# Joao-M-Silva/padel_analytics

Hardware: AMD Instinct MI355X
Metric: frames/sec (all trackers) on 1280x720 (higher is better)
Workload: dtype f32-equivalent (h2: fp16 pairs h + m/2048, 2 or 3 f16 MFMA products per multiply, fp32 accumulate)

## Files before the change

padel_analytics_amd/csrc/conv_1x1_h2s.hip:

```cpp
#include "h2_common.h"

namespace padel {

namespace {

}

#ifndef PADEL_HS_AWIN
#define PADEL_HS_AWIN D
#endif
template <int WC, int PROBE = 0, int D = 2, int WR = 2>
__global__ void __launch_bounds__(64 * WR * WC, 2) conv_h2s_kernel(const ConvArgs a) {
    constexpr int MF = 4, NF = 3, NSET = D + 1;
    constexpr int kSPlaneB = 64 * WR * 64;
    constexpr int kSStageB = 2 * kSPlaneB;
    constexpr int kSStages = WC == 2 ? 5 : 9;
    constexpr int kSAhead = kSStages - 1;
    constexpr int NA = 8 / (2 * WC) * 2;
    static_assert(WR == 2 || WC == 4, "64-pixel tiles: one span per wave");
    __shared__ __attribute__((aligned(16))) float lds[(kSStages * kSStageB) / 4];
    char* const ldsb = reinterpret_cast<char*>(lds);
    const int tid = threadIdx.x;
    const int lane = tid & 63;
    const int wave = __builtin_amdgcn_readfirstlane(tid >> 6);
    const int wr = WR == 2 ? (wave & 1) : 0, wc = WR == 2 ? (wave >> 1) : wave;
    const int lr = lane & 15, lq = lane >> 4;

    const int nmt = a.n_mtiles, nnt = a.n_ntiles;
    const int bid = blockIdx.x;
    const XcdSlot slot = xcd_slot(nmt, nnt, bid);
    if (xcd_slot_padding(slot)) return;
    const int mt = xcd_slot_mtile(slot), nt = slot.nt;
    const int m0 = mt * (64 * WR);
    const int f0 = nt * WC * NF;
    const int nch = a.cin >> 5;

    const long long pix_b = (long long)a.in_cs * 4;
    const char* const in0 = reinterpret_cast<const char*>(a.in + a.in_choff) + (long long)m0 * pix_b;
    i32x4 rsrcA = make_rsrc(in0);
    {
        const long long left = ((long long)a.M - m0) * pix_b;
        rsrcA[2] = (int)(left > 0x7FFFFFFFll ? 0x7FFFFFFFll : left);
    }
    const int p_q = (lane & 3) ^ (((lane >> 4) & 1) << 1);
    const unsigned p_piece = (unsigned)((p_q >> 1) * 64 + (p_q & 1) * 16);
    unsigned voA[2];
#pragma unroll
    for (int k = 0; k < 2; ++k) voA[k] = (unsigned)(((wave + 4 * k) * 16 + (lane >> 2)) * (unsigned)pix_b) + p_piece;
    unsigned voL[2];
#pragma unroll
    for (int k = 0; k < 2; ++k) voL[k] = (unsigned)((wave * 16 + 8 * k + (lane >> 3)) * (unsigned)pix_b) + (unsigned)(lane & 7) * 16u;
    i32x4 sink[2] = {};
    unsigned voQ[2];
#pragma unroll
    for (int k = 0; k < 2; ++k) voQ[k] = (unsigned)(wave * 2048 + k * 1024 + lane * 16);
    const unsigned lp0 = __builtin_amdgcn_readfirstlane((unsigned)(uintptr_t)lds);
    const unsigned lpw = __builtin_amdgcn_readfirstlane(lp0 + (unsigned)wave * 1024u);
#define PADEL_HS_REQA(SB_, K_)                                                                                    \
    if constexpr (PROBE != 3) {                                                                                   \
        const unsigned so_ = (unsigned)(K_) * 128u;                                                               \
        const unsigned lb_ = lpw + (unsigned)(SB_);                                                               \
        i32x4 rs_ = rsrcA;                                                                                        \
        if ((int)(K_) >= nch) rs_[2] = 0;                                                                         \
        if constexpr (PROBE == 4) { lds_dma<0>(voL[0], rs_, so_, lb_); lds_dma<kSPlaneB>(voL[1], rs_, so_, lb_); } \
        else if constexpr (PROBE == 6) {                                                                          \
            asm volatile("buffer_load_dwordx4 %0, %1, %2, %3 offen" : "=v"(sink[0]) : "v"(voA[0]), "s"(rs_), "s"(so_) : "memory"); \
            asm volatile("buffer_load_dwordx4 %0, %1, %2, %3 offen" : "=v"(sink[1]) : "v"(voA[0]), "s"(rs_), "s"(so_ + 32u) : "memory"); \
        }                                                                                                         \
        else if constexpr (PROBE == 5) { lds_dma<0>(voQ[0], rs_, so_ * 128u, lb_); lds_dma<kSPlaneB>(voQ[1], rs_, so_ * 128u, lb_); } \
        else {                                                                                                    \
        lds_dma<0>(voA[0], rs_, so_, lb_); if constexpr (WC == 2) lds_dma<4096>(voA[1], rs_, so_, lb_);           \
        lds_dma<kSPlaneB>(voA[0], rs_, so_ + 32u, lb_); if constexpr (WC == 2) lds_dma<kSPlaneB + 4096>(voA[1], rs_, so_ + 32u, lb_); \
        }                                                                                                         \
    }

    const unsigned fragb = (unsigned)nch * 2048u;
    const unsigned voffW = (unsigned)lane * 16u;
    i32x4 rsrcW[NF];
#pragma unroll
    for (int j = 0; j < NF; ++j) {
        const int frag = min(f0 + NF * wc + j, a.n16 - 1);
        rsrcW[j] = make_rsrc(reinterpret_cast<const char*>(a.wr) + (long long)frag * fragb);
    }
    i32x4 w[NSET][NF];
#define PADEL_HS_LOADW(SET_, K_)                                                                                  \
    if constexpr (PROBE != 2 && PROBE < 4 || PROBE == 7) {                                                        \
        const unsigned so_ = (unsigned)(K_) * 2048u;                                                              \
        if (PROBE == 7 && wr == 1) rsrcW[0][2] = rsrcW[1][2] = rsrcW[2][2] = 0;      \
        _Pragma("unroll") for (int j = 0; j < NF; ++j)                                                            \
            asm volatile("buffer_load_dwordx4 %0, %1, %2, %3 offen" : "=v"(w[SET_][j]) : "v"(voffW), "s"(rsrcW[j]), "s"(so_) : "memory"); \
    }
#define PADEL_HS_WAITW(SET_, N_)                                                                                  \
    asm volatile("s_waitcnt vmcnt(%3)" : "+v"(w[SET_][0]), "+v"(w[SET_][1]), "+v"(w[SET_][2]) : "n"(PROBE == 2 || (PROBE >= 4 && PROBE != 7) ? ((N_) == 0 ? 0 : (PADEL_HS_AWIN) * NA) : PROBE == 3 ? (N_) * NF / (NF + NA) : (N_)) : "memory")

    const unsigned abase = swz_off(64 * wr + lr, lq);
    f32x4 acc[MF][NF], part[MF][NF], cross[MF][NF];
#pragma unroll
    for (int f = 0; f < MF; ++f)
#pragma unroll
        for (int j = 0; j < NF; ++j) { acc[f][j] = (f32x4){0.f, 0.f, 0.f, 0.f}; part[f][j] = acc[f][j]; cross[f][j] = acc[f][j]; }
    h16x8 ah[MF], am[MF];
#define PADEL_HS_MFMA(F_, SET_)                                                                                   \
    do {                                                                                                          \
        _Pragma("unroll") for (int j = 0; j < NF; ++j)                                                            \
            cross[F_][j] = __builtin_amdgcn_mfma_f32_16x16x32_f16(__builtin_bit_cast(h16x8, w[SET_][j]), am[F_], cross[F_][j], 0, 0, 0); \
        _Pragma("unroll") for (int j = 0; j < NF; ++j)                                                            \
            part[F_][j] = __builtin_amdgcn_mfma_f32_16x16x32_f16(__builtin_bit_cast(h16x8, w[SET_][j]), ah[F_], part[F_][j], 0, 0, 0); \
        __builtin_amdgcn_sched_barrier(0);                                                                        \
    } while (0)
#define PADEL_HS_STEP(K_, SET_)                                                                                   \
    do {                                                                                                          \
        PADEL_HS_LOADW(((SET_) + D) % NSET, (K_) + D);                                                            \
        PADEL_HS_WAITW(SET_, D * (NF + NA));                                                                      \
        __builtin_amdgcn_s_barrier();              \
        asm volatile("" ::: "memory");                                                                            \
        PADEL_HS_REQA(s_wr, (K_) + kSAhead);                                                                      \
        __builtin_amdgcn_sched_barrier(0);                                                                        \
        if constexpr (PROBE == 0) {                                                                               \
            const char* p_ = ldsb + abase + s_rd;                                                                 \
            _Pragma("unroll") for (int f = 0; f < MF; ++f) {                                                      \
                ah[f] = *reinterpret_cast<const h16x8*>(p_ + f * 1024);                                           \
                am[f] = *reinterpret_cast<const h16x8*>(p_ + f * 1024 + kSPlaneB);                                \
            }                                                                                                     \
        }                                                                                                         \
        __builtin_amdgcn_sched_barrier(0);                                                                        \
        if constexpr (PROBE == 0) { PADEL_HS_MFMA(0, SET_); PADEL_HS_MFMA(1, SET_); PADEL_HS_MFMA(2, SET_); PADEL_HS_MFMA(3, SET_); } \
        if (++kblk == 9) {                         \
            kblk = 0;                                                                                             \
            _Pragma("unroll") for (int f = 0; f < MF; ++f)                                                        \
                _Pragma("unroll") for (int j = 0; j < NF; ++j) { acc[f][j] += part[f][j]; part[f][j] = (f32x4){0.f, 0.f, 0.f, 0.f}; } \
        }                                                                                                         \
        s_wr = s_rd;                                                                                              \
        s_rd = s_rd + (unsigned)kSStageB == (unsigned)(kSStages * kSStageB) ? 0u : s_rd + (unsigned)kSStageB;     \
    } while (0)

    int kblk = 0;
    unsigned s_rd = 0, s_wr = (unsigned)((kSStages - 1) * kSStageB);
    static_assert(kSAhead >= D, "the ring is at least as deep as the weight look-ahead");
#pragma unroll
    for (int k = 0; k < kSAhead - D; ++k) PADEL_HS_REQA(k * kSStageB, k);
#pragma unroll
    for (int i = 0; i < D; ++i) {
        PADEL_HS_LOADW(i, i);
        PADEL_HS_REQA((kSAhead - D + i) * kSStageB, kSAhead - D + i);
    }
#pragma unroll 1
    for (int k = 0; k < nch; k += NSET) {
        PADEL_HS_STEP(k, 0);
#pragma unroll
        for (int i = 1; i < NSET; ++i)
            if (k + i < nch) PADEL_HS_STEP(k + i, i);
    }
    if (kblk != 0) {
#pragma unroll
        for (int f = 0; f < MF; ++f)
#pragma unroll
            for (int j = 0; j < NF; ++j) acc[f][j] += part[f][j];
    }
#pragma unroll
    for (int i = 0; i < NSET; ++i) PADEL_HS_WAITW(i, 0);
    if constexpr (PROBE == 6) asm volatile("" :: "v"(sink[0]), "v"(sink[1]));
#undef PADEL_HS_STEP
#undef PADEL_HS_MFMA
#undef PADEL_HS_WAITW
#undef PADEL_HS_LOADW
#undef PADEL_HS_REQA

    int mpix[MF];
#pragma unroll
    for (int f = 0; f < MF; ++f) {
        const int m = m0 + 64 * wr + 16 * f + lr;
        mpix[f] = m < a.M ? m : -1;
    }
    const int fw = f0 + NF * wc;
    const bool fast = m0 + 64 * WR <= a.M && (fw + NF) * 16 <= a.cout && (((a.out_choff | a.out_cs) & 3) == 0) &&
                      (!a.res || (((a.res_choff | a.res_cs) & 3) == 0));
    if (fw < a.n16) h2_epilogue<MF, NF>(a, acc, cross, mpix, fw, lq, fast);
}

template <int PROBE = 0, int WR = 2>
__global__ void __launch_bounds__(256 * WR, 2) conv_h2s3_kernel(const ConvArgs a) {
    constexpr int MF = 4, NF = 3, WC = 4;
    constexpr int kSPlaneB = 64 * WR * 64, kSStageB = 2 * kSPlaneB;
    constexpr int kSStages = 9, kSAhead = 8, NA = 2;
    __shared__ __attribute__((aligned(16))) float lds[(kSStages * kSStageB) / 4];
    char* const ldsb = reinterpret_cast<char*>(lds);
    const int tid = threadIdx.x;
    const int lane = tid & 63;
    const int wave = __builtin_amdgcn_readfirstlane(tid >> 6);
    const int wr = WR == 2 ? (wave & 1) : 0, wc = WR == 2 ? (wave >> 1) : wave;
    const int lr = lane & 15, lq = lane >> 4;

    const int nmt = a.n_mtiles, nnt = a.n_ntiles;
    const int bid = blockIdx.x;
    const XcdSlot slot = xcd_slot(nmt, nnt, bid);
    if (xcd_slot_padding(slot)) return;
    const int mt = xcd_slot_mtile(slot), nt = slot.nt;
    const int m0 = mt * (64 * WR);
    const int f0 = nt * WC * NF;
    const int nch = a.cin >> 5;
    const int HoWo = a.Ho * a.Wo;

    const long long pix_b = (long long)a.in_cs * 4;
    long long lin0;
    {
        const int n = fastdiv(m0, a.howo_magic, a.howo_shift);
        const int rem = m0 - n * HoWo;
        const int oy = fastdiv(rem, a.wo_magic, a.wo_shift), ox = rem - oy * a.Wo;
        lin0 = ((long long)n * a.H + (2 * oy - 1)) * a.W + (2 * ox - 1);
    }
    const i32x4 rsrcA = make_rsrc(reinterpret_cast<const char*>(a.in + a.in_choff) + lin0 * pix_b);
    const int p_q = (lane & 3) ^ (((lane >> 4) & 1) << 1);
    const unsigned p_piece = (unsigned)((p_q >> 1) * 64 + (p_q & 1) * 16);
    unsigned voA, vbits = 0;
    {
        const int m = m0 + wave * 16 + (lane >> 2);
        const bool mv = m < a.M;
        const int mc = mv ? m : m0;
        const int n = fastdiv(mc, a.howo_magic, a.howo_shift);
        const int rem = mc - n * HoWo;
        const int oy = fastdiv(rem, a.wo_magic, a.wo_shift), ox = rem - oy * a.Wo;
        const int iy0 = 2 * oy - 1, ix0 = 2 * ox - 1;
        const long long lin = ((long long)n * a.H + iy0) * a.W + ix0;
        voA = (unsigned)((lin - lin0) * pix_b) + p_piece;
        if (mv) {
#pragma unroll
            for (int k = 0; k < 3; ++k) {
                vbits |= ((unsigned)(iy0 + k) < (unsigned)a.H ? 1u : 0u) << k;
                vbits |= ((unsigned)(ix0 + k) < (unsigned)a.W ? 8u : 0u) << k;
            }
        }
    }
    const unsigned rowb = (unsigned)a.W * (unsigned)pix_b;
    const unsigned lp0 = __builtin_amdgcn_readfirstlane((unsigned)(uintptr_t)lds);
    const unsigned lpw = __builtin_amdgcn_readfirstlane(lp0 + (unsigned)wave * 1024u);
#define PADEL_HS3_REQA(SB_, CH_, TAP_)                                                                            \
    do {                                                                                                          \
        constexpr int ky_ = (TAP_) % 3, kx_ = (TAP_) / 3;                                                         \
        constexpr unsigned need_ = (1u << ky_) | (8u << kx_);                                                     \
        const unsigned so_ = (unsigned)(CH_) * 128u + (unsigned)ky_ * rowb + (unsigned)kx_ * (unsigned)pix_b;     \
        const unsigned lb_ = lpw + (unsigned)(SB_);                                                               \
        i32x4 rs_ = rsrcA;                                                                                        \
        if ((int)(CH_) >= nch) rs_[2] = 0;                                                                        \
        const unsigned vo_ = (vbits & need_) == need_ ? voA : kOOR;                                               \
        lds_dma<0>(vo_, rs_, so_, lb_); lds_dma<kSPlaneB>(vo_, rs_, so_ + 32u, lb_);                              \
    } while (0)

    const unsigned fragb = (unsigned)(nch * 9) * 2048u;
    const unsigned voffW = (unsigned)lane * 16u;
    i32x4 rsrcW[NF];
#pragma unroll
    for (int j = 0; j < NF; ++j) {
        const int frag = min(f0 + NF * wc + j, a.n16 - 1);
        rsrcW[j] = make_rsrc(reinterpret_cast<const char*>(a.wr) + (long long)frag * fragb);
    }
    i32x4 w[3][NF];
    unsigned s_kw = 0;
#define PADEL_HS3_LOADW(SET_, TT_)                                                                                \
    do {                                                                                                          \
        const unsigned so_ = s_kw + (unsigned)((TT_) * 2048);                                                     \
        _Pragma("unroll") for (int j = 0; j < NF; ++j)                                                            \
            asm volatile("buffer_load_dwordx4 %0, %1, %2, %3 offen" : "=v"(w[SET_][j]) : "v"(voffW), "s"(rsrcW[j]), "s"(so_) : "memory"); \
    } while (0)
#define PADEL_HS3_WAITW(SET_, N_)                                                                                 \
    asm volatile("s_waitcnt vmcnt(%3)" : "+v"(w[SET_][0]), "+v"(w[SET_][1]), "+v"(w[SET_][2]) : "n"(N_) : "memory")

    const unsigned abase = swz_off(64 * wr + lr, lq);
    f32x4 acc[MF][NF], part[MF][NF], cross[MF][NF];
#pragma unroll
    for (int f = 0; f < MF; ++f)
#pragma unroll
        for (int j = 0; j < NF; ++j) { acc[f][j] = (f32x4){0.f, 0.f, 0.f, 0.f}; part[f][j] = acc[f][j]; cross[f][j] = acc[f][j]; }
    h16x8 ah[MF], am[MF];
#define PADEL_HS3_MFMA(F_, SET_)                                                                                  \
    do {                                                                                                          \
        _Pragma("unroll") for (int j = 0; j < NF; ++j)                                                            \
            cross[F_][j] = __builtin_amdgcn_mfma_f32_16x16x32_f16(__builtin_bit_cast(h16x8, w[SET_][j]), am[F_], cross[F_][j], 0, 0, 0); \
        _Pragma("unroll") for (int j = 0; j < NF; ++j)                                                            \
            part[F_][j] = __builtin_amdgcn_mfma_f32_16x16x32_f16(__builtin_bit_cast(h16x8, w[SET_][j]), ah[F_], part[F_][j], 0, 0, 0); \
        __builtin_amdgcn_sched_barrier(0);                                                                        \
    } while (0)
#define PADEL_HS3_STEP(T_)                                                                                        \
    do {                                                                                                          \
        PADEL_HS3_LOADW(((T_) + 2) % 3, (T_) + 2);                                                                \
        PADEL_HS3_WAITW((T_) % 3, 2 * NF + 2 * NA);                                                               \
        __builtin_amdgcn_s_barrier();                                                                             \
        asm volatile("" ::: "memory");                                                                            \
        PADEL_HS3_REQA(s_wr, c + ((T_) >= 1 ? 1 : 0), ((T_) + 8) % 9);                                            \
        __builtin_amdgcn_sched_barrier(0);                                                                        \
        if constexpr (PROBE == 0) {                                                                               \
            const char* p_ = ldsb + abase + s_rd;                                                                 \
            _Pragma("unroll") for (int f = 0; f < MF; ++f) {                                                      \
                ah[f] = *reinterpret_cast<const h16x8*>(p_ + f * 1024);                                           \
                am[f] = *reinterpret_cast<const h16x8*>(p_ + f * 1024 + kSPlaneB);                                \
            }                                                                                                     \
        }                                                                                                         \
        __builtin_amdgcn_sched_barrier(0);                                                                        \
        if constexpr (PROBE == 0) { PADEL_HS3_MFMA(0, (T_) % 3); PADEL_HS3_MFMA(1, (T_) % 3); PADEL_HS3_MFMA(2, (T_) % 3); PADEL_HS3_MFMA(3, (T_) % 3); } \
        s_wr = s_rd;                                                                                              \
        s_rd = s_rd + (unsigned)kSStageB == (unsigned)(kSStages * kSStageB) ? 0u : s_rd + (unsigned)kSStageB;     \
    } while (0)

    unsigned s_rd = 0, s_wr = (unsigned)((kSStages - 1) * kSStageB);
    PADEL_HS3_REQA(0 * kSStageB, 0, 0); PADEL_HS3_REQA(1 * kSStageB, 0, 1);
    PADEL_HS3_REQA(4 * kSStageB, 0, 4); PADEL_HS3_REQA(5 * kSStageB, 0, 5); PADEL_HS3_REQA(6 * kSStageB, 0, 6); PADEL_HS3_REQA(7 * kSStageB, 0, 7);
    PADEL_HS3_LOADW(0, 0);
    PADEL_HS3_REQA(2 * kSStageB, 0, 2);
    PADEL_HS3_LOADW(1, 1);
    PADEL_HS3_REQA(3 * kSStageB, 0, 3);
#pragma unroll 1
    for (int c = 0; c < nch; ++c) {
        PADEL_HS3_STEP(0); PADEL_HS3_STEP(1); PADEL_HS3_STEP(2); PADEL_HS3_STEP(3); PADEL_HS3_STEP(4);
        PADEL_HS3_STEP(5); PADEL_HS3_STEP(6); PADEL_HS3_STEP(7); PADEL_HS3_STEP(8);
#pragma unroll
        for (int f = 0; f < MF; ++f)
#pragma unroll
            for (int j = 0; j < NF; ++j) { acc[f][j] += part[f][j]; part[f][j] = (f32x4){0.f, 0.f, 0.f, 0.f}; }
        s_kw += 9u * 2048u;
    }
    PADEL_HS3_WAITW(0, 0); PADEL_HS3_WAITW(1, 0); PADEL_HS3_WAITW(2, 0);
#undef PADEL_HS3_STEP
#undef PADEL_HS3_MFMA
#undef PADEL_HS3_WAITW
#undef PADEL_HS3_LOADW
#undef PADEL_HS3_REQA

    int mpix[MF];
#pragma unroll
    for (int f = 0; f < MF; ++f) {
        const int m = m0 + 64 * wr + 16 * f + lr;
        mpix[f] = m < a.M ? m : -1;
    }
    const int fw = f0 + NF * wc;
    const bool fast = m0 + 64 * WR <= a.M && (fw + NF) * 16 <= a.cout && (((a.out_choff | a.out_cs) & 3) == 0) &&
                      (!a.res || (((a.res_choff | a.res_cs) & 3) == 0));
    if (fw < a.n16) h2_epilogue<MF, NF>(a, acc, cross, mpix, fw, lq, fast);
}

hipError_t launch_conv_h2s3(const ConvArgs& a_in, int tile, hipStream_t s) {
    if (tile != 246 && tile != 248) return hipErrorNotSupported;
    const bool m64 = tile == 248;
    ConvArgs a = a_in;
    a.n_mtiles = m64 ? (a.M + 63) / 64 : (a.M + 127) / 128;
    a.n_ntiles = (a.n16 + 11) / 12;
    dim3 grid(8u * (unsigned)((a.n_mtiles + 7) / 8) * (unsigned)a.n_ntiles, 1, 1);
    if (m64) {
        if (a.tune & 64) hipLaunchKernelGGL((conv_h2s3_kernel<1, 1>), grid, dim3(256), 0, s, a);
        else hipLaunchKernelGGL((conv_h2s3_kernel<0, 1>), grid, dim3(256), 0, s, a);
        return hipGetLastError();
    }
    if (a.tune & 64) hipLaunchKernelGGL((conv_h2s3_kernel<1>), grid, dim3(512), 0, s, a);
    else hipLaunchKernelGGL((conv_h2s3_kernel<0>), grid, dim3(512), 0, s, a);
    return hipGetLastError();
}

hipError_t launch_conv_h2s(const ConvArgs& a_in, int tile, hipStream_t s) {
    if (tile != 244 && tile != 245 && tile != 247) return hipErrorNotSupported;
    const bool nf12 = tile != 244, m64 = tile == 247;
    ConvArgs a = a_in;
    if (nf12 && m64) {
        a.n_mtiles = (a.M + 63) / 64;
        a.n_ntiles = (a.n16 + 11) / 12;
        dim3 grid(8u * (unsigned)((a.n_mtiles + 7) / 8) * (unsigned)a.n_ntiles, 1, 1);
        if (a.tune & 64) hipLaunchKernelGGL((conv_h2s_kernel<4, 1, 2, 1>), grid, dim3(256), 0, s, a);
        else hipLaunchKernelGGL((conv_h2s_kernel<4, 0, 2, 1>), grid, dim3(256), 0, s, a);
        return hipGetLastError();
    }
    a.n_mtiles = (a.M + 127) / 128;
    const bool wide = nf12;
    a.n_ntiles = wide ? (a.n16 + 11) / 12 : (a.n16 + 5) / 6;
    dim3 grid(8u * (unsigned)((a.n_mtiles + 7) / 8) * (unsigned)a.n_ntiles, 1, 1);
    if (wide) {
        static bool attr = false;
        if (!attr) {
            (void)hipFuncSetAttribute(reinterpret_cast<const void*>(conv_h2s_kernel<4, 0>), hipFuncAttributeMaxDynamicSharedMemorySize, 0);
            attr = true;
        }
        if ((a.tune & 64) && (a.tune & 4096)) hipLaunchKernelGGL((conv_h2s_kernel<4, 7>), grid, dim3(512), 0, s, a);
        else if ((a.tune & 64) && (a.tune & 2048)) hipLaunchKernelGGL((conv_h2s_kernel<4, 6>), grid, dim3(512), 0, s, a);
        else if ((a.tune & 64) && (a.tune & 1024)) hipLaunchKernelGGL((conv_h2s_kernel<4, 5>), grid, dim3(512), 0, s, a);
        else if ((a.tune & 64) && (a.tune & 256) && (a.tune & 512)) hipLaunchKernelGGL((conv_h2s_kernel<4, 4>), grid, dim3(512), 0, s, a);
        else if ((a.tune & 64) && (a.tune & 256)) hipLaunchKernelGGL((conv_h2s_kernel<4, 2>), grid, dim3(512), 0, s, a);
        else if ((a.tune & 64) && (a.tune & 512)) hipLaunchKernelGGL((conv_h2s_kernel<4, 3>), grid, dim3(512), 0, s, a);
        else if (a.tune & 64) hipLaunchKernelGGL((conv_h2s_kernel<4, 1>), grid, dim3(512), 0, s, a);
        else if (a.tune & 8) hipLaunchKernelGGL((conv_h2s_kernel<4, 0, 4>), grid, dim3(512), 0, s, a);
        else hipLaunchKernelGGL((conv_h2s_kernel<4, 0, 2>), grid, dim3(512), 0, s, a);
    } else if (a.tune & 64) hipLaunchKernelGGL((conv_h2s_kernel<2, 1>), grid, dim3(256), 0, s, a);
    else if (a.tune & 8) hipLaunchKernelGGL((conv_h2s_kernel<2, 0, 3>), grid, dim3(256), 0, s, a);
    else hipLaunchKernelGGL((conv_h2s_kernel<2, 0, 2>), grid, dim3(256), 0, s, a);
    return hipGetLastError();
}

}
```

padel_analytics_amd/csrc/h2_common.h:

```cpp
#pragma once
#include "kernels.h"
#include "conv_prims.h"
#include <cmath>
#include "act_fast.h"

namespace padel {

namespace {

constexpr float kH2Max = 65504.0f;
constexpr float kH2Scale = 2048.0f, kH2InvScale = 1.0f / 2048.0f;
constexpr unsigned kOORh = 0x80000000u;

__device__ __forceinline__ long long h2_chan_off(int c) { return (long long)(c >> 4) * 64 + (c & 15) * 2; }

__device__ __forceinline__ void h2_encode4(const f32x4 v, h16x4& h, h16x4& m, bool& bad) {
#pragma unroll
    for (int p = 0; p < 2; ++p) {
        bad = bad || !(fabsf(v[2 * p]) <= kH2Max) || !(fabsf(v[2 * p + 1]) <= kH2Max);
        const f32x2 x = {__builtin_amdgcn_fmed3f(v[2 * p], -kH2Max, kH2Max), __builtin_amdgcn_fmed3f(v[2 * p + 1], -kH2Max, kH2Max)};
        const h16x2 hh = __builtin_convertvector(x, h16x2);
        const f32x2 rr = {(x[0] - (float)hh[0]) * kH2Scale, (x[1] - (float)hh[1]) * kH2Scale};
        const h16x2 mm = __builtin_convertvector(rr, h16x2);
        h[2 * p] = hh[0]; h[2 * p + 1] = hh[1];
        m[2 * p] = mm[0]; m[2 * p + 1] = mm[1];
    }
}

template <int ACT>
__device__ __forceinline__ float h2_act(float x) { return fast_act<ACT>(x); }
__device__ __forceinline__ f32x4 h2_decode4(const h16x4 h, const h16x4 m) {
    f32x4 v;
#pragma unroll
    for (int r = 0; r < 4; ++r) v[r] = fmaf((float)m[r], kH2InvScale, (float)h[r]);
    return v;
}
__device__ __forceinline__ void h2_raise(unsigned* flag, bool bad) {
    if (__builtin_amdgcn_ballot_w64(bad) != 0ull && (threadIdx.x & 63) == 0) atomicOr(flag, 1u);
}

}

typedef unsigned short h2_u16x2 __attribute__((ext_vector_type(2)));

__device__ __forceinline__ float h2_conv_value(float cross, float mainacc, float sc, float b) {
    return fmaf(fmaf(cross, kH2InvScale, mainacc), sc, b);
}
__device__ __forceinline__ f32x4 h2_residual4(const u32x4 rr) {
    const u32x2 s0 = __builtin_amdgcn_permlane16_swap(rr[0], rr[2], false, false);
    const u32x2 s1 = __builtin_amdgcn_permlane16_swap(rr[1], rr[3], false, false);
    const u32x2 hd = {s0[0], s1[0]}, md = {s0[1], s1[1]};
    return h2_decode4(__builtin_bit_cast(h16x4, hd), __builtin_bit_cast(h16x4, md));
}

template <int MF, int NF, int ACT, bool RES, bool F32OUT>
__device__ __forceinline__ void h2_epilogue_fast(const ConvArgs& a, const f32x4 (&mainacc)[MF][NF], const f32x4 (&cross)[MF][NF],
                                                 const int (&mpix)[MF], int fw, int lq, bool& bad) {
    static_assert(!(RES && F32OUT), "fp32 head maps have no residual");
    f32x4 b[NF], sc[NF];
#pragma unroll
    for (int j = 0; j < NF; ++j) {
        const int co0 = (fw + j) * 16 + lq * 4;
        b[j] = *reinterpret_cast<const f32x4*>(a.bias + co0);
        sc[j] = *reinterpret_cast<const f32x4*>(a.oscale + co0);
    }
    if constexpr (F32OUT) {
        float* op[MF];
#pragma unroll
        for (int f = 0; f < MF; ++f) op[f] = a.out + (long long)mpix[f] * a.out_cs + (a.out_choff + fw * 16 + lq * 4);
#pragma unroll
        for (int j = 0; j < NF; ++j)
#pragma unroll
            for (int f = 0; f < MF; ++f) {
                f32x4 v;
#pragma unroll
                for (int r = 0; r < 4; ++r) v[r] = h2_act<ACT>(h2_conv_value(cross[f][j][r], mainacc[f][j][r], sc[j][r], b[j][r]));
                *reinterpret_cast<f32x4*>(op[f] + j * 16) = v;
            }
    } else {
        const int piece = ((lq & 1) << 5) | ((lq >> 1) << 4);
        char* op[MF];
        u32x4 rr[MF][NF];
#pragma unroll
        for (int f = 0; f < MF; ++f) {
            op[f] = reinterpret_cast<char*>(a.out) + (long long)mpix[f] * a.out_cs * 4 + ((((a.out_choff >> 4) + fw) << 6) + piece);
            if constexpr (RES) {
                const char* rp = reinterpret_cast<const char*>(a.res) + (long long)mpix[f] * a.res_cs * 4 + ((((a.res_choff >> 4) + fw) << 6) + piece);
#pragma unroll
                for (int j = 0; j < NF; ++j) rr[f][j] = *reinterpret_cast<const u32x4*>(rp + j * 64);
            }
        }
        h2_u16x2 top = {0, 0};
#pragma unroll
        for (int j = 0; j < NF; ++j)
#pragma unroll
            for (int f = 0; f < MF; ++f) {
                f32x4 v;
#pragma unroll
                for (int r = 0; r < 4; ++r) v[r] = h2_conv_value(cross[f][j][r], mainacc[f][j][r], sc[j][r], b[j][r]);
                if constexpr (RES) {
                    const f32x4 rv = h2_residual4(rr[f][j]);
                    if (a.res_pre) {
#pragma unroll
                        for (int r = 0; r < 4; ++r) v[r] = h2_act<ACT>(v[r] + rv[r]);
                    } else {
#pragma unroll
                        for (int r = 0; r < 4; ++r) v[r] = h2_act<ACT>(v[r]) + rv[r];
                    }
                } else {
#pragma unroll
                    for (int r = 0; r < 4; ++r) v[r] = h2_act<ACT>(v[r]);
                }
                u32x2 hd, md;
#pragma unroll
                for (int p = 0; p < 2; ++p) {
                    const f32x2 x = {__builtin_amdgcn_fmed3f(v[2 * p], -kH2Max, kH2Max), __builtin_amdgcn_fmed3f(v[2 * p + 1], -kH2Max, kH2Max)};
                    const h16x2 hh = __builtin_convertvector(x, h16x2);
                    const f32x2 res = {(x[0] - (float)hh[0]) * kH2Scale, (x[1] - (float)hh[1]) * kH2Scale};
                    const h16x2 mm = __builtin_convertvector(res, h16x2);
                    hd[p] = __builtin_bit_cast(unsigned, hh);
                    md[p] = __builtin_bit_cast(unsigned, mm);
                    top = __builtin_elementwise_max(top, __builtin_bit_cast(h2_u16x2, hd[p] & 0x7FFF7FFFu));
                }
                const u32x2 s0 = __builtin_amdgcn_permlane16_swap(hd[0], md[0], false, false);
                const u32x2 s1 = __builtin_amdgcn_permlane16_swap(hd[1], md[1], false, false);
                const u32x4 o = {s0[0], s1[0], s0[1], s1[1]};
                *reinterpret_cast<u32x4*>(op[f] + j * 64) = o;
            }
        bad = bad || top[0] >= 0x7BFFu || top[1] >= 0x7BFFu;
    }
}

template <int MF, int NF, int ACT, bool RES>
__device__ __forceinline__ void h2_epilogue_slow(const ConvArgs& a, const f32x4 (&mainacc)[MF][NF], const f32x4 (&cross)[MF][NF],
                                                 const int (&mpix)[MF], int fw, int lq, bool& bad) {
    char* const outb = reinterpret_cast<char*>(a.out);
    const char* const resb = reinterpret_cast<const char*>(a.res);
#pragma unroll
    for (int j = 0; j < NF; ++j) {
        const int co0 = (fw + j) * 16 + lq * 4;
        f32x4 b, sc;
#pragma unroll
        for (int r = 0; r < 4; ++r) { b[r] = a.bias[min(co0 + r, a.n16 * 16 - 1)]; sc[r] = a.oscale[min(co0 + r, a.n16 * 16 - 1)]; }
#pragma unroll
        for (int f = 0; f < MF; ++f) {
            const int m = mpix[f];
            if (m < 0) continue;
#pragma unroll
            for (int r = 0; r < 4; ++r) {
                const int co = co0 + r;
                if (co >= a.cout) continue;
                float x = h2_conv_value(cross[f][j][r], mainacc[f][j][r], sc[r], b[r]);
                if (RES) {
                    const int rc = a.res_choff + co;
                    const _Float16* rp = reinterpret_cast<const _Float16*>(resb + (long long)m * a.res_cs * 4 + (long long)(rc >> 4) * 64) + (rc & 15);
                    const float rv = fmaf((float)rp[16], kH2InvScale, (float)rp[0]);
                    x = a.res_pre ? h2_act<ACT>(x + rv) : h2_act<ACT>(x) + rv;
                } else {
                    x = h2_act<ACT>(x);
                }
                if (a.out_f32) {
                    a.out[(long long)m * a.out_cs + a.out_choff + co] = x;
                } else {
                    bad |= !(fabsf(x) <= kH2Max);
                    const float xc = __builtin_amdgcn_fmed3f(x, -kH2Max, kH2Max);
                    const _Float16 hh = (_Float16)xc;
                    const int oc = a.out_choff + co;
                    _Float16* op = reinterpret_cast<_Float16*>(outb + (long long)m * a.out_cs * 4 + (long long)(oc >> 4) * 64) + (oc & 15);
                    op[0] = hh;
                    op[16] = (_Float16)((xc - (float)hh) * kH2Scale);
                }
            }
        }
    }
}

template <int MF, int NF>
__device__ __forceinline__ void h2_epilogue(const ConvArgs& a, const f32x4 (&mainacc)[MF][NF], const f32x4 (&cross)[MF][NF],
                                            const int (&mpix)[MF], int fw, int lq, bool fast) {
    const bool wide = fast && (a.out_f32 ? !a.res : ((((a.out_choff | a.out_cs) & 15) == 0) && (!a.res || (((a.res_choff | a.res_cs) & 15) == 0))));
    bool bad = false;
#define PADEL_H2_EPI(ACT_)                                                                                        \
    do {                                                                                                          \
        if (wide) {                                                                                               \
            if (a.out_f32) h2_epilogue_fast<MF, NF, ACT_, false, true>(a, mainacc, cross, mpix, fw, lq, bad);     \
            else if (a.res) h2_epilogue_fast<MF, NF, ACT_, true, false>(a, mainacc, cross, mpix, fw, lq, bad);    \
            else h2_epilogue_fast<MF, NF, ACT_, false, false>(a, mainacc, cross, mpix, fw, lq, bad);              \
        } else if (a.res) h2_epilogue_slow<MF, NF, ACT_, true>(a, mainacc, cross, mpix, fw, lq, bad);             \
        else h2_epilogue_slow<MF, NF, ACT_, false>(a, mainacc, cross, mpix, fw, lq, bad);                         \
    } while (0)
    if (a.act == ACT_SILU) PADEL_H2_EPI(ACT_SILU);
    else if (a.act == ACT_RELU) PADEL_H2_EPI(ACT_RELU);
    else if (a.act == ACT_SIGMOID) PADEL_H2_EPI(ACT_SIGMOID);
    else if (a.act == ACT_LEAKY) PADEL_H2_EPI(ACT_LEAKY);
    else PADEL_H2_EPI(ACT_NONE);
#undef PADEL_H2_EPI
    if (!a.out_f32) h2_raise(a.ovf_flag, bad);
}

}
```

Before: 1026.

## Add persistent tile-walking 1x1 h2 conv kernel with cross-tile activation prefetch

Adds a persistent kernel for the wide (nf12) 1x1 h2 conv. It launches about one or two blocks per CU, and each block walks a strided sequence of output tiles. The activation DMA ring keeps prefetching into the next tile, so loads overlap the previous tile's MFMA and epilogue work. Bias and scale are staged once into LDS so the epilogue does no global loads while requests are in flight, and partial sums are flushed every 9 k-blocks. The path is used only when there is no residual, cin/32 is divisible by 3, and the grid is large enough. It adds LDS use and complexity, and the fixed walk order may load-balance worse than a full grid.

```diff
diff --git a/padel_analytics_amd/csrc/conv_1x1_h2s.hip b/padel_analytics_amd/csrc/conv_1x1_h2s.hip
--- a/padel_analytics_amd/csrc/conv_1x1_h2s.hip
+++ b/padel_analytics_amd/csrc/conv_1x1_h2s.hip
@@ -178,6 +178,178 @@
     if (fw < a.n16) h2_epilogue<MF, NF>(a, acc, cross, mpix, fw, lq, fast);
 }
 
+struct HsWalk { int mloc, nt; };
+template <int BM>
+__device__ __forceinline__ i32x4 hs_rsrc(const ConvArgs& a, int mt, bool valid) {
+    const long long pix_b = (long long)a.in_cs * 4;
+    const int m0 = valid ? mt * BM : 0;
+    i32x4 r = make_rsrc(reinterpret_cast<const char*>(a.in + a.in_choff) + (long long)m0 * pix_b);
+    const unsigned long long left = (unsigned long long)(((long long)a.M - m0) * pix_b);
+    r[2] = valid ? ((left >> 31) != 0ull ? 0x7FFFFFFF : (int)(unsigned)left) : 0;
+    return r;
+}
+
+template <int WR>
+__global__ void __launch_bounds__(256 * WR, 2) conv_h2s_kernel_walk(const ConvArgs a) {
+    constexpr int MF = 4, NF = 3, WC = 4, D = 2, NSET = D + 1, NA = 2;
+    constexpr int BM = 64 * WR;
+    constexpr int kSPlaneB = BM * 64, kSStageB = 2 * kSPlaneB;
+    constexpr int kSStages = 9, kSAhead = kSStages - 1;
+    constexpr int kRingB = kSStages * kSStageB;
+    __shared__ __attribute__((aligned(16))) float lds[(kRingB + 2 * kH2LdsVecB) / 4];
+    char* const ldsb = reinterpret_cast<char*>(lds);
+    const int tid = threadIdx.x;
+    const int lane = tid & 63;
+    const int wave = __builtin_amdgcn_readfirstlane(tid >> 6);
+    const int wr = WR == 2 ? (wave & 1) : 0, wc = WR == 2 ? (wave >> 1) : wave;
+    const int lr = lane & 15, lq = lane >> 4;
+    const int nch = a.cin >> 5;
+    const int nnt = a.n_ntiles;
+    const XcdSlot slot0 = xcd_slot(a.n_mtiles, nnt, (int)blockIdx.x);
+    if (xcd_slot_padding(slot0)) return;
+    const int mlim = slot0.q8 + (slot0.xcd < slot0.r8 ? 1 : 0);
+    const int xbase = xcd_slot_mtile(slot0) - slot0.mloc;
+    const int gs = (int)gridDim.x >> 3;
+    const int dq = gs / nnt, dr = gs - dq * nnt;
+#define PADEL_HSW_NEXT(W_) do { (W_).mloc += dq; (W_).nt += dr; if ((W_).nt >= nnt) { (W_).nt -= nnt; ++(W_).mloc; } } while (0)
+    HsWalk cur = {slot0.mloc, slot0.nt};
+
+    const unsigned pix_b = (unsigned)a.in_cs * 4u;
+    const int p_q = (lane & 3) ^ (((lane >> 4) & 1) << 1);
+    const unsigned voA = (unsigned)(wave * 16 + (lane >> 2)) * pix_b + (unsigned)((p_q >> 1) * 64 + (p_q & 1) * 16);
+    const unsigned lp0 = __builtin_amdgcn_readfirstlane((unsigned)(uintptr_t)lds);
+    const unsigned lpw = __builtin_amdgcn_readfirstlane(lp0 + (unsigned)wave * 1024u);
+    const unsigned ldsv = lp0 + (unsigned)kRingB;
+    HsWalk rq = cur;
+    int rq_k = 0;
+    i32x4 rq_rs = hs_rsrc<BM>(a, xbase + rq.mloc, true);
+#define PADEL_HSW_REQA(SB_)                                                                                       \
+    do {                                                                                                          \
+        const unsigned so_ = (unsigned)rq_k * 128u;                                                               \
+        const unsigned lb_ = lpw + (unsigned)(SB_);                                                               \
+        lds_dma<0>(voA, rq_rs, so_, lb_);                                                                         \
+        lds_dma<kSPlaneB>(voA, rq_rs, so_ + 32u, lb_);                                                            \
+        if (++rq_k == nch) {                                                                                      \
+            rq_k = 0;                                                                                             \
+            PADEL_HSW_NEXT(rq);                                                                                   \
+            rq_rs = hs_rsrc<BM>(a, xbase + rq.mloc, rq.mloc < mlim);                                              \
+        }                                                                                                         \
+    } while (0)
+
+    const unsigned fragb = (unsigned)nch * 2048u;
+    const unsigned voffW = (unsigned)lane * 16u;
+    i32x4 rsrcW[NF];
+    i32x4 w[NSET][NF];
+#define PADEL_HSW_LOADW(SET_, K_)                                                                                 \
+    do {                                                                                                          \
+        const unsigned so_ = (unsigned)(K_) * 2048u;                                                              \
+        _Pragma("unroll") for (int j = 0; j < NF; ++j)                                                            \
+            asm volatile("buffer_load_dwordx4 %0, %1, %2, %3 offen" : "=v"(w[SET_][j]) : "v"(voffW), "s"(rsrcW[j]), "s"(so_) : "memory"); \
+    } while (0)
+#define PADEL_HSW_PUBLISH(SET_) asm volatile("" : "+v"(w[SET_][0]), "+v"(w[SET_][1]), "+v"(w[SET_][2]) :: "memory")
+
+    const unsigned abase = swz_off(64 * wr + lr, lq);
+    f32x4 acc[MF][NF], part[MF][NF], cross[MF][NF];
+    h16x8 ah[MF], am[MF];
+#define PADEL_HSW_MFMA(F_, SET_)                                                                                  \
+    do {                                                                                                          \
+        _Pragma("unroll") for (int j = 0; j < NF; ++j)                                                            \
+            cross[F_][j] = __builtin_amdgcn_mfma_f32_16x16x32_f16(__builtin_bit_cast(h16x8, w[SET_][j]), am[F_], cross[F_][j], 0, 0, 0); \
+        _Pragma("unroll") for (int j = 0; j < NF; ++j)                                                            \
+            part[F_][j] = __builtin_amdgcn_mfma_f32_16x16x32_f16(__builtin_bit_cast(h16x8, w[SET_][j]), ah[F_], part[F_][j], 0, 0, 0); \
+        __builtin_amdgcn_sched_barrier(0);                                                                        \
+    } while (0)
+#define PADEL_HSW_STEP(P_)                                                                                        \
+    do {                                                                                                          \
+        if ((P_) == 0 || !last) PADEL_HSW_LOADW(((P_) + D) % NSET, k + (P_) + D);                                 \
+        if constexpr ((P_) == 0) { if (k == 0) wait_vm<2 * NF>(); else wait_vm<2 * (NF + NA)>(); }                \
+        else if constexpr ((P_) == 1) {                                                                           \
+            if (k == 0) { if (last) wait_vm<NF + NA>(); else wait_vm<2 * NF + NA>(); }                            \
+            else { if (last) wait_vm<NF + 2 * NA>(); else wait_vm<2 * (NF + NA)>(); }                             \
+        } else { if (last) wait_vm<2 * NA>(); else wait_vm<2 * (NF + NA)>(); }                                    \
+        PADEL_HSW_PUBLISH(P_);                                                                                    \
+        __builtin_amdgcn_s_barrier();              \
+        asm volatile("" ::: "memory");                                                                            \
+        PADEL_HSW_REQA(s_wr);                                                                                     \
+        __builtin_amdgcn_sched_barrier(0);                                                                        \
+        {                                                                                                         \
+            const char* p_ = ldsb + abase + s_rd;                                                                 \
+            _Pragma("unroll") for (int f = 0; f < MF; ++f) {                                                      \
+                ah[f] = *reinterpret_cast<const h16x8*>(p_ + f * 1024);                                           \
+                am[f] = *reinterpret_cast<const h16x8*>(p_ + f * 1024 + kSPlaneB);                                \
+            }                                                                                                     \
+        }                                                                                                         \
+        __builtin_amdgcn_sched_barrier(0);                                                                        \
+        PADEL_HSW_MFMA(0, P_); PADEL_HSW_MFMA(1, P_); PADEL_HSW_MFMA(2, P_); PADEL_HSW_MFMA(3, P_);               \
+        if (++kblk == 9) {                         \
+            kblk = 0;                                                                                             \
+            _Pragma("unroll") for (int f = 0; f < MF; ++f)                                                        \
+                _Pragma("unroll") for (int j = 0; j < NF; ++j) { acc[f][j] += part[f][j]; part[f][j] = (f32x4){0.f, 0.f, 0.f, 0.f}; } \
+        }                                                                                                         \
+        s_wr = s_rd;                                                                                              \
+        s_rd = s_rd + (unsigned)kSStageB == (unsigned)kRingB ? 0u : s_rd + (unsigned)kSStageB;                    \
+    } while (0)
+
+    {
+        unsigned sb = 0;
+#pragma unroll 1
+        for (int k = 0; k < kSAhead; ++k, sb += (unsigned)kSStageB) PADEL_HSW_REQA(sb);
+    }
+    {
+        float* const vb = lds + kRingB / 4;
+        for (int i = tid; i < a.n16 * 16; i += 256 * WR) { vb[i] = a.bias[i]; vb[kH2LdsVecB / 4 + i] = a.oscale[i]; }
+        lds_fence();
+    }
+    unsigned s_rd = 0, s_wr = (unsigned)((kSStages - 1) * kSStageB);
+    for (;;) {
+#pragma unroll
+        for (int j = 0; j < NF; ++j) {
+            const int frag = min(cur.nt * (WC * NF) + NF * wc + j, a.n16 - 1);
+            rsrcW[j] = make_rsrc(reinterpret_cast<const char*>(a.wr) + (long long)frag * fragb);
+        }
+        PADEL_HSW_LOADW(0, 0);
+        PADEL_HSW_LOADW(1, 1);
+#pragma unroll
+        for (int f = 0; f < MF; ++f)
+#pragma unroll
+            for (int j = 0; j < NF; ++j) { acc[f][j] = (f32x4){0.f, 0.f, 0.f, 0.f}; part[f][j] = acc[f][j]; cross[f][j] = acc[f][j]; }
+        int kblk = 0;
+#pragma unroll 1
+        for (int k = 0; k < nch; k += NSET) {
+            const bool last = k + NSET >= nch;
+            PADEL_HSW_STEP(0); PADEL_HSW_STEP(1); PADEL_HSW_STEP(2);
+        }
+        if (kblk != 0) {
+#pragma unroll
+            for (int f = 0; f < MF; ++f)
+#pragma unroll
+                for (int j = 0; j < NF; ++j) acc[f][j] += part[f][j];
+        }
+        const int m0 = (xbase + cur.mloc) * BM;
+        int lane_e = lane;
+        asm volatile("" : "+v"(lane_e));
+        const int lr_e = lane_e & 15, lq_e = lane_e >> 4;
+        int mpix[MF];
+#pragma unroll
+        for (int f = 0; f < MF; ++f) {
+            const int m = m0 + 64 * wr + 16 * f + lr_e;
+            mpix[f] = m < a.M ? m : -1;
+        }
+        const int fw = cur.nt * (WC * NF) + NF * wc;
+        const bool fast = m0 + BM <= a.M && (fw + NF) * 16 <= a.cout && (((a.out_choff | a.out_cs) & 3) == 0);
+        if (fw < a.n16) h2_epilogue<MF, NF, true>(a, acc, cross, mpix, fw, lq_e, fast, ldsv);
+        PADEL_HSW_NEXT(cur);
+        if (cur.mloc >= mlim) break;
+    }
+    wait_vm<0>();
+#undef PADEL_HSW_STEP
+#undef PADEL_HSW_MFMA
+#undef PADEL_HSW_PUBLISH
+#undef PADEL_HSW_LOADW
+#undef PADEL_HSW_REQA
+#undef PADEL_HSW_NEXT
+}
+
 template <int PROBE = 0, int WR = 2>
 __global__ void __launch_bounds__(256 * WR, 2) conv_h2s3_kernel(const ConvArgs a) {
     constexpr int MF = 4, NF = 3, WC = 4;
@@ -358,6 +530,27 @@
     if (tile != 244 && tile != 245 && tile != 247) return hipErrorNotSupported;
     const bool nf12 = tile != 244, m64 = tile == 247;
     ConvArgs a = a_in;
+    if (nf12) {
+        a.n_mtiles = m64 ? (a.M + 63) / 64 : (a.M + 127) / 128;
+        a.n_ntiles = (a.n16 + 11) / 12;
+        const int vmax = 8 * ((a.n_mtiles + 7) / 8) * a.n_ntiles;
+        static int n_cu = 0;
+        if (!n_cu) { int dev = 0; hipDeviceProp_t p; if (hipGetDevice(&dev) == hipSuccess && hipGetDeviceProperties(&p, dev) == hipSuccess) n_cu = p.multiProcessorCount; if (n_cu <= 0) n_cu = 256; }
+        const int cap = ((m64 ? 2 : 1) * n_cu) & ~7;
+        const bool walk = !(a.tune & (4 | 8 | 64)) && !a.res && a.wr && (a.cin >> 5) % 3 == 0 && a.n16 * 16 * 4 <= kH2LdsVecB &&
+                          cap >= 8 && vmax >= 2 * cap;
+        if (walk) {
+            static bool attr = false;
+            if (!attr) {
+                (void)hipFuncSetAttribute(reinterpret_cast<const void*>(conv_h2s_kernel_walk<1>), hipFuncAttributeMaxDynamicSharedMemorySize, 0);
+                (void)hipFuncSetAttribute(reinterpret_cast<const void*>(conv_h2s_kernel_walk<2>), hipFuncAttributeMaxDynamicSharedMemorySize, 0);
+                attr = true;
+            }
+            if (m64) hipLaunchKernelGGL((conv_h2s_kernel_walk<1>), dim3((unsigned)cap), dim3(256), 0, s, a);
+            else hipLaunchKernelGGL((conv_h2s_kernel_walk<2>), dim3((unsigned)cap), dim3(512), 0, s, a);
+            return hipGetLastError();
+        }
+    }
     if (nf12 && m64) {
         a.n_mtiles = (a.M + 63) / 64;
         a.n_ntiles = (a.n16 + 11) / 12;
diff --git a/padel_analytics_amd/csrc/h2_common.h b/padel_analytics_amd/csrc/h2_common.h
--- a/padel_analytics_amd/csrc/h2_common.h
+++ b/padel_analytics_amd/csrc/h2_common.h
@@ -53,16 +53,25 @@
     return h2_decode4(__builtin_bit_cast(h16x4, hd), __builtin_bit_cast(h16x4, md));
 }
 
-template <int MF, int NF, int ACT, bool RES, bool F32OUT>
+constexpr int kH2LdsVecB = 4096;
+typedef __attribute__((address_space(3))) const f32x4 h2_lds_f32x4;
+typedef __attribute__((address_space(3))) const float h2_lds_f32;
+template <int MF, int NF, int ACT, bool RES, bool F32OUT, bool LDSV = false>
 __device__ __forceinline__ void h2_epilogue_fast(const ConvArgs& a, const f32x4 (&mainacc)[MF][NF], const f32x4 (&cross)[MF][NF],
-                                                 const int (&mpix)[MF], int fw, int lq, bool& bad) {
+                                                 const int (&mpix)[MF], int fw, int lq, bool& bad, unsigned ldsv = 0) {
     static_assert(!(RES && F32OUT), "fp32 head maps have no residual");
+    static_assert(!(RES && LDSV), "a residual is a global load: not for kernels that keep requests in flight across the epilogue");
     f32x4 b[NF], sc[NF];
 #pragma unroll
     for (int j = 0; j < NF; ++j) {
         const int co0 = (fw + j) * 16 + lq * 4;
-        b[j] = *reinterpret_cast<const f32x4*>(a.bias + co0);
-        sc[j] = *reinterpret_cast<const f32x4*>(a.oscale + co0);
+        if constexpr (LDSV) {
+            b[j] = *reinterpret_cast<h2_lds_f32x4*>(ldsv + (unsigned)co0 * 4u);
+            sc[j] = *reinterpret_cast<h2_lds_f32x4*>(ldsv + (unsigned)kH2LdsVecB + (unsigned)co0 * 4u);
+        } else {
+            b[j] = *reinterpret_cast<const f32x4*>(a.bias + co0);
+            sc[j] = *reinterpret_cast<const f32x4*>(a.oscale + co0);
+        }
     }
     if constexpr (F32OUT) {
         float* op[MF];
@@ -131,9 +140,9 @@
     }
 }
 
-template <int MF, int NF, int ACT, bool RES>
+template <int MF, int NF, int ACT, bool RES, bool LDSV = false>
 __device__ __forceinline__ void h2_epilogue_slow(const ConvArgs& a, const f32x4 (&mainacc)[MF][NF], const f32x4 (&cross)[MF][NF],
-                                                 const int (&mpix)[MF], int fw, int lq, bool& bad) {
+                                                 const int (&mpix)[MF], int fw, int lq, bool& bad, unsigned ldsv = 0) {
     char* const outb = reinterpret_cast<char*>(a.out);
     const char* const resb = reinterpret_cast<const char*>(a.res);
 #pragma unroll
@@ -141,7 +150,15 @@
         const int co0 = (fw + j) * 16 + lq * 4;
         f32x4 b, sc;
 #pragma unroll
-        for (int r = 0; r < 4; ++r) { b[r] = a.bias[min(co0 + r, a.n16 * 16 - 1)]; sc[r] = a.oscale[min(co0 + r, a.n16 * 16 - 1)]; }
+        for (int r = 0; r < 4; ++r) {
+            const int cc = min(co0 + r, a.n16 * 16 - 1);
+            if constexpr (LDSV) {
+                b[r] = *reinterpret_cast<h2_lds_f32*>(ldsv + (unsigned)cc * 4u);
+                sc[r] = *reinterpret_cast<h2_lds_f32*>(ldsv + (unsigned)kH2LdsVecB + (unsigned)cc * 4u);
+            } else {
+                b[r] = a.bias[cc]; sc[r] = a.oscale[cc];
+            }
+        }
 #pragma unroll
         for (int f = 0; f < MF; ++f) {
             const int m = mpix[f];
@@ -173,6 +190,28 @@
             }
         }
     }
+}
+
+template <int MF, int NF, bool LDSV>
+__device__ __forceinline__ void h2_epilogue(const ConvArgs& a, const f32x4 (&mainacc)[MF][NF], const f32x4 (&cross)[MF][NF],
+                                            const int (&mpix)[MF], int fw, int lq, bool fast, unsigned ldsv) {
+    static_assert(LDSV, "the global-load form takes no LDS offset");
+    const bool wide = fast && (a.out_f32 || (((a.out_choff | a.out_cs) & 15) == 0));
+    bool bad = false;
+#define PADEL_H2_EPI(ACT_)                                                                                        \
+    do {                                                                                                          \
+        if (wide) {                                                                                               \
+            if (a.out_f32) h2_epilogue_fast<MF, NF, ACT_, false, true, true>(a, mainacc, cross, mpix, fw, lq, bad, ldsv); \
+            else h2_epilogue_fast<MF, NF, ACT_, false, false, true>(a, mainacc, cross, mpix, fw, lq, bad, ldsv);  \
+        } else h2_epilogue_slow<MF, NF, ACT_, false, true>(a, mainacc, cross, mpix, fw, lq, bad, ldsv);           \
+    } while (0)
+    if (a.act == ACT_SILU) PADEL_H2_EPI(ACT_SILU);
+    else if (a.act == ACT_RELU) PADEL_H2_EPI(ACT_RELU);
+    else if (a.act == ACT_SIGMOID) PADEL_H2_EPI(ACT_SIGMOID);
+    else if (a.act == ACT_LEAKY) PADEL_H2_EPI(ACT_LEAKY);
+    else PADEL_H2_EPI(ACT_NONE);
+#undef PADEL_H2_EPI
+    if (!a.out_f32) h2_raise(a.ovf_flag, bad);
 }
 
 template <int MF, int NF>
```

Result: no change. 1028 (median of 6 runs) (+0.2%).
